# Liupeter01/Software-Rasterizer

Measured on AMD Instinct MI355X. Metric: frames_per_sec, higher is better.
Workload: dtype f32

## Files before the change

software-rasterizer_amd/csrc/srz_api.hip:

```cpp
#include <dlfcn.h>

#include <algorithm>
#include <cmath>
#include <cstdio>
#include <cstdlib>
#include <cstring>
#include <initializer_list>
#include <new>
#include <string>
#include <vector>

#include "srz_device.h"

using namespace srz;

namespace {
std::string g_create_error;

struct EventPair {
  hipEvent_t t0, t1, t2, t3;
  bool detailed;
};

struct BatchDesc {
// ... 82 lines not shown
  bool tris_aos = false;
  BBox *d_bbox = nullptr;
  uint16_t *d_tri_batch = nullptr;
  srz_light *d_lights = nullptr;
  uint32_t *d_pool = nullptr;
  uint32_t pool_sub_cap = 0, pool_n_sub = 1;
  bool pool_sized = false;
  uint32_t *d_pool_heads = nullptr, *h_pool_heads = nullptr;
  static constexpr int DEMAND_PARTS = 8;
  uint2 *d_tile_info = nullptr;
  uint32_t last_flags = 0;
  bool rendered = false;
  uint32_t *d_sparse_rows = nullptr;
  uint32_t *d_slow_list = nullptr, *d_slow_count = nullptr;
  uint4 *d_redo_list = nullptr;
  uint32_t fast_kinds = 0;
  bool any_generic = true;
  uint32_t *d_vis = nullptr, *d_work_count = nullptr, *d_chunk_rows = nullptr;
  uint4 *d_worklist = nullptr;
  uint64_t kind_slots = 0;
  uint32_t kind_mask = 0, n_kind_slots = 0;
  bool approx_shade = false;
  bool no_packed = false;
  uint32_t *d_band_desc = nullptr;
  uint2 *d_band_ent = nullptr;
  uint64_t total_groups = 0;
  ShadeDescG *d_sdesc = nullptr;
  DrawDesc *d_draws = nullptr;
  static constexpr int STAGE_RING = 4;
  uint8_t *d_dyn = nullptr;
// ... 110 lines not shown
  (void)hipFree(fs->d_dyn);
  (void)hipFree(fs->d_tris);
  (void)hipFree(fs->d_tri_pos);
  (void)hipFree(fs->d_bbox);
  (void)hipFree(fs->d_tri_batch);
  (void)hipFree(fs->d_pool);
  (void)hipFree(fs->d_pool_heads);
  if (fs->h_pool_heads) (void)hipHostFree(fs->h_pool_heads);
  if (fs->clear_tune.h_wgs) (void)hipHostFree(fs->clear_tune.h_wgs), fs->clear_tune.h_wgs = nullptr;
  if (fs->clear_tune.d_ctl) (void)hipFree(fs->clear_tune.d_ctl), fs->clear_tune.d_ctl = nullptr;
  (void)hipFree(fs->d_tile_info);
  (void)hipFree(fs->d_sparse_rows);
  (void)hipFree(fs->d_slow_list);
  (void)hipFree(fs->d_slow_count);
  (void)hipFree(fs->d_redo_list);
  (void)hipFree(fs->d_vis);
  (void)hipFree(fs->d_worklist);
  (void)hipFree(fs->d_work_count);
  (void)hipFree(fs->d_chunk_rows);
  (void)hipFree(fs->d_band_desc);
  (void)hipFree(fs->d_band_ent);
  (void)hipFree(fs->d_sdesc);
}

struct Pass {
  enum Kind { COLOUR, VISIBILITY, COUNTING, SIZE_ONLY, PEEL } kind = COLOUR;
  int f_begin = 0, f_count = -1;
  bool one_frame_scratch = false;
  const float *d_prev = nullptr;
  static Pass colour() { return {}; }
// ... 23 lines not shown
  a.bbox = fs->d_bbox;
  a.chunk_rows = fs->d_chunk_rows;
  a.band_desc = fs->d_band_desc;
  a.band_ent = fs->d_band_ent;
  a.tri_batch = fs->d_tri_batch;
  a.lights = fs->d_lights;
  a.pool = fs->d_pool;
  a.pool_heads = fs->d_pool_heads;
  a.pool_demand = fs->h_pool_heads;
  a.pool_sub_cap = fs->pool_sub_cap;
  a.pool_sub_mask = fs->pool_n_sub - 1u;
  a.tile_info = fs->d_tile_info;
  a.slow_list = fs->d_slow_list;
  a.slow_count = fs->d_slow_count;
  a.redo_list = fs->d_redo_list;
  a.redo_count = fs->d_slow_count + 1;
  a.force_ordered = a.force_generic = pass.kind == Pass::COUNTING ? 1u : 0u;
  a.any_ordered = any_frame_has(fs, flags_or, SRZ_ORDERED_RASTER) ? 1u : 0u, a.any_generic = fs->any_generic ? 1u : 0u;
  a.sdesc = fs->d_sdesc;
  a.vis = fs->d_vis;
  a.worklist = fs->d_worklist;
  a.kind_slots = fs->kind_slots;
  a.work_count = fs->d_work_count;
  a.work_cap = (uint32_t)(fs->n_frames < 8 ? fs->n_frames : (fs->n_frames + 7) / 8) * fs->n_local_bands * fs->tiles_x;
  a.tiles_x = fs->tiles_x;
  a.n_local_bands = fs->n_local_bands;
  a.n_frames = (uint32_t)fs->n_frames;
  a.out = d_out;
  a.local_rows = fs->local_rows;
  a.frame_stride = pass.one_frame_scratch ? 0 : 4ull * fs->local_rows * (uint64_t)fs->width;
// ... 836 lines not shown
    fs->pool_n_sub = n_sub;
    const uint64_t cap = std::min<uint64_t>((4ull * tri_off + 4096u) / n_sub + 64u, 0xfffffff0ull / n_sub);
    fs->pool_sub_cap = (uint32_t)cap;
    FS_TRY(dev_alloc((void **)&fs->d_pool, sizeof(uint32_t) * cap * n_sub));
    FS_TRY(dev_alloc((void **)&fs->d_pool_heads, sizeof(uint32_t) * CNT_STRIDE * 64));
    FS_TRY(hipHostMalloc((void **)&fs->h_pool_heads, sizeof(uint32_t) * CNT_STRIDE * 64 * srz_frameset::DEMAND_PARTS, hipHostMallocMapped | hipHostMallocCoherent));
    if (e == hipSuccess) std::memset(fs->h_pool_heads, 0, sizeof(uint32_t) * CNT_STRIDE * 64 * srz_frameset::DEMAND_PARTS);
    FS_TRY(dev_alloc((void **)&fs->clear_tune.d_ctl, sizeof(ClearCtl)));
    if (e == hipSuccess) FS_TRY(hipMemset(fs->clear_tune.d_ctl, 0, sizeof(ClearCtl)));
    FS_TRY(hipHostMalloc((void **)&fs->clear_tune.h_wgs, 64, hipHostMallocMapped | hipHostMallocCoherent));
    if (e == hipSuccess) *fs->clear_tune.h_wgs = 0u;
    FS_TRY(dev_alloc((void **)&fs->d_tile_info, sizeof(uint2) * fs->max_tiles));
    FS_TRY(dev_alloc((void **)&fs->d_slow_list, sizeof(uint32_t) * fs->max_tiles));
    FS_TRY(dev_alloc((void **)&fs->d_slow_count, 2 * sizeof(uint32_t)));
    FS_TRY(dev_alloc((void **)&fs->d_redo_list, sizeof(uint4) * fs->max_tiles));
  }
  FS_TRY(dev_alloc((void **)&fs->d_vis, sizeof(uint32_t) * (size_t)fs->max_tiles * ((size_t)TILE * TILE)));
  FS_TRY(ensure_worklists(fs));
  FS_TRY(dev_alloc((void **)&fs->d_work_count, sizeof(uint32_t) * CNT_STRIDE * N_WORK_LISTS));
  FS_TRY(dev_alloc((void **)&fs->d_sdesc, sizeof(ShadeDescG) * fs->h_batches.size()));
  std::vector<uint8_t> h_dyn(fs->dyn_bytes);
  stage_dyn(fs, h_dyn.data());
  FS_TRY(hipMemcpy(fs->d_dyn, h_dyn.data(), fs->dyn_bytes, hipMemcpyHostToDevice));
  if (tri_off) {
    if (copy_tris) FS_TRY(hipMemcpy(fs->d_tris, h_tris.data(), sizeof(srz_tri) * tri_off, hipMemcpyHostToDevice));
    if (!h_pos.empty()) FS_TRY(hipMemcpy(fs->d_tri_pos, h_pos.data(), sizeof(float) * h_pos.size(), hipMemcpyHostToDevice));
    FS_TRY(hipMemcpy(fs->d_tri_batch, h_tb.data(), sizeof(uint16_t) * tri_off, hipMemcpyHostToDevice));
  }
#undef FS_TRY
  if (e != hipSuccess) {
// ... 402 lines not shown
  if (!fs || !d_vis || !d_out) return fail(ctx, SRZ_E_INVALID, fn + ": null frameset / visibility buffer / output");
  const size_t bytes = srz_frameset_out_bytes(ctx, fs);
  if (out_bytes < bytes) return fail(ctx, SRZ_E_INVALID, fn + ": output buffer too small");
  if (!aligned<16>({d_vis, d_out})) return fail(ctx, SRZ_E_INVALID, fn + ": buffers must be 16-byte aligned");
  if (d_vis != d_out && ranges_overlap({d_vis, bytes}, {d_out, bytes}))
    return fail(ctx, SRZ_E_INVALID, fn + ": visibility buffer and output overlap partly");
  hipStream_t s;
  if (int rc = begin_pass(ctx, fs, stream, PASS_SHADING | PASS_VERTEX, &s)) return rc;
  ShadeVisArgs a{};
  fill_walk(a, fs, d_vis, d_out);
  a.tris = fs->d_tris, a.tri_batch = fs->d_tri_batch, a.lights = fs->d_lights, a.sdesc = fs->d_sdesc;
  a.frame_stride = 4ull * plane_words(fs);
  a.flags_or = flags & FRAME_FLAGS, a.in_place = d_vis == d_out ? 1u : 0u;
  a.any_generic = fs->any_generic ? 1u : 0u;
  a.redo_list = reinterpret_cast<uint32_t *>(fs->d_redo_list), a.redo_count = fs->d_slow_count + 1;
  HIP_TRY(ctx, hipMemsetAsync(a.redo_count, 0, sizeof(uint32_t), s));
  launch_shade_vis(a, fs->fast_kinds, fs->any_generic, fs->approx_shade, s);
  const srz_frameset::ClearTune &ct = fs->clear_tune;
  if (!ctx->env_clear_wgs && ct.d_ctl && !ct.done && fs->max_tiles >= 8192) launch_clear_rebase(ct.d_ctl, s);
  return end_pass(ctx);
}

size_t srz_frameset_gbuffer_bytes(const srz_ctx *ctx, const srz_frameset *fs, uint32_t what) {
  if (!fs || what == 0u || (what & ~GB_GROUPS) != 0u) return 0;
  return (size_t)fs->n_frames * gbuf_planes(what) * fs->local_rows * (size_t)fs->width * sizeof(float);
}

int srz_frameset_gbuffer(srz_ctx *ctx, srz_frameset *fs, const void *d_vis, void *d_out, size_t out_bytes, uint32_t what, uint32_t flags,
                         void *stream) {
  if (!ctx) return SRZ_E_INVALID;
// ... 2069 lines not shown
```

software-rasterizer_amd/csrc/srz_device.h:

```cpp
#pragma once
#include <hip/hip_runtime.h>
#include <stdint.h>

#include "../../include/srz.h"

namespace srz {

constexpr int TILE = 32;
constexpr int BAND = 32;
constexpr int KEY_STRIDE = TILE + 1;
constexpr int LDS_STRIDE = 32;
#ifndef SRZ_BAND_ROT
#define SRZ_BAND_ROT 5
#endif
__host__ __device__ inline int band_rot(int world) { return (SRZ_BAND_ROT % world) ? SRZ_BAND_ROT : (SRZ_BAND_ROT ? 1 : 0); }
__host__ __device__ inline int band_of(int lb, int rank, int world) {
  if (world == 1) return lb;
  int j = (rank - band_rot(world) * lb) % world;
  return lb * world + (j < 0 ? j + world : j);
}
__host__ __device__ inline int rank_of_band(int b, int world) { return (b + band_rot(world) * (b / world)) % world; }
constexpr uint32_t NO_TRI = 0xffffffffu;
constexpr uint32_t CNT_STRIDE = 32;
constexpr uint32_t FD_FAST_SHADE = 0x100u, FD_NL_SHIFT = 9;
// ... 76 lines not shown
  uint32_t *pool;
  uint32_t *pool_heads;
  uint32_t *pool_demand;
  uint32_t pool_sub_cap, pool_sub_mask;
  uint2 *tile_info;
  uint32_t *slow_list;
  uint32_t *slow_count;
  uint32_t other_streams;
  uint32_t clear_in_raster;
  uint32_t force_ordered;
  uint32_t any_ordered;
  uint32_t force_generic;
  uint32_t any_generic;
  uint4 *redo_list;
  uint32_t *redo_count;
  uint32_t *vis;
  uint4 *worklist;
  uint64_t kind_slots;
  uint32_t *work_count;
  uint32_t work_cap;
  uint32_t tiles_x, n_local_bands, n_frames;
  float *out;
  uint64_t frame_stride;
  uint32_t local_rows;
  int32_t shard_rank, shard_world;
  uint32_t flags_or;
  unsigned long long *stats;
  const uint32_t *clear_wgs_dev;
};

// ... 82 lines not shown
struct ShadeVisArgs {
  const FrameDesc *frames;
  const srz_tri *tris;
  const uint16_t *tri_batch;
  const srz_light *lights;
  const ShadeDescG *sdesc;
  const float *vis;
  float *out;
  uint64_t frame_stride;
  uint32_t local_rows, tiles_x, n_local_bands, n_frames;
  int32_t shard_rank, shard_world;
  uint32_t flags_or, in_place;
  uint32_t any_generic;
  uint32_t *redo_list;
  uint32_t *redo_count;
};
void launch_shade_vis(const ShadeVisArgs &a, uint32_t kinds, bool any_generic, bool approx, hipStream_t s);
struct GbufArgs {
  const FrameDesc *frames;
  const srz_tri *tris;
  const uint16_t *tri_batch;
  const ShadeDescG *sdesc;
  const float *vis;
  float *out;
  uint64_t vis_stride;
  uint64_t frame_stride;
  uint32_t local_rows, tiles_x, n_local_bands, n_frames;
  int32_t shard_rank, shard_world;
  uint32_t flags_or, what;
};
// ... 443 lines not shown
```

software-rasterizer_amd/csrc/srz_kernels.hip:

```cpp
#include "srz_device.h"

#include <algorithm>
#include <cstdio>
#include <cstdlib>
#include <type_traits>

#pragma clang fp contract(off)

namespace srz {

#define SRZ_CAS __attribute__((address_space(4)))
template <typename T> __device__ __forceinline__ const SRZ_CAS T *as_const(const T *p) { return (const SRZ_CAS T *)(p); }
typedef float f32x4 __attribute__((ext_vector_type(4)));
typedef unsigned int u32x2 __attribute__((ext_vector_type(2)));
typedef unsigned int u32x4 __attribute__((ext_vector_type(4)));

__device__ __forceinline__ float sse_max(float a, float b) { return a > b ? a : b; }
__device__ __forceinline__ float sse_min(float a, float b) { return a < b ? a : b; }
__device__ __forceinline__ float std_max(float a, float b) { return (a < b) ? b : a; }
__device__ __forceinline__ float std_clamp(float v, float lo, float hi) { return (v < lo) ? lo : (hi < v) ? hi : v; }
__device__ __forceinline__ float fmsubf(float a, float b, float c) { return __builtin_fmaf(a, b, -c); }
__device__ __forceinline__ float fmaf_(float a, float b, float c) { return __builtin_fmaf(a, b, c); }

__device__ __forceinline__ uint32_t f2u_(float f) { return __builtin_bit_cast(uint32_t, f); }
// ... 2263 lines not shown

#ifndef SRZ_FAST_MINW
#define SRZ_FAST_MINW 6
#endif
#ifndef SRZ_STAGE_TRIS
#define SRZ_STAGE_TRIS 96
#endif
constexpr uint32_t STAGE_TRIS = SRZ_STAGE_TRIS, STAGE_SD = 16;
static_assert(SRZ_STAGE_TRIS * 6 * 16 >= 2 * 32 * 32 * 4, "SRZ_STAGE_TRIS: s_tri must hold a tile's 1024 {pixel, index} pairs (>= 86 triangles)");
#ifndef SRZ_GENPOW_MINW
#define SRZ_GENPOW_MINW 5
#endif
#ifndef SRZ_SHADE_MINW
#define SRZ_SHADE_MINW 4
#endif
template <bool STATS, int FASTNL, bool BUMPY = false, bool APPROX = false>
__global__ __launch_bounds__(256, (FASTNL > 0 && FASTNL <= 2 && !BUMPY) ? SRZ_FAST_MINW : (FASTNL < 0 && FASTNL >= -2) ? SRZ_GENPOW_MINW
                                  : ((FASTNL == 3 || FASTNL == -3) && !BUMPY) ? 5 : SRZ_SHADE_MINW)
void k_shade(RenderArgs a) {
  constexpr bool FAST = FASTNL != 0, GENPOW = FASTNL < 0;
  static_assert(FAST || !BUMPY, "BUMPY is a property of the FAST builds");
  static_assert(!APPROX || (FASTNL > 0 && !BUMPY && !STATS), "the tolerance mode has FAST builds for 1..4 lights only");
  static_assert(!(GENPOW && BUMPY), "frames with BUMP / DISPLACEMENT batches and a non-integer exponent take the generic build");
  __shared__ __attribute__((aligned(16))) float s_c[3][TILE * TILE];
  __shared__ __attribute__((aligned(16))) uint32_t s_ent[PIX_SLOT];
  __shared__ uint32_t s_wcnt[4];
  __shared__ __attribute__((aligned(16))) f32x4 s_tri[STAGE_TRIS * 6];
  __shared__ uint16_t s_bat[STAGE_TRIS];
  __shared__ __attribute__((aligned(16))) ShadeDescG s_sd[STAGE_SD];
  __shared__ uint32_t s_flag;

  const int tid = threadIdx.x, lane = tid & 63;
  const int wave = __builtin_amdgcn_readfirstlane(tid >> 6);
  unsigned long long n_vis = 0, n_vis_tex = 0;
#ifdef SRZ_PHASE_PROBE
  unsigned long long ph[6] = {0, 0, 0, 0, 0, 0}, ph_t = 0;
  const unsigned long long ph_c0 = __builtin_amdgcn_s_memtime(), ph_r0 = __builtin_amdgcn_s_memrealtime();
#define SRZ_STAMP(K) { const unsigned long long t_ = __builtin_amdgcn_s_memtime(); ph[K] += t_ - ph_t, ph_t = t_; }
#else
#define SRZ_STAMP(K)
#endif

  auto shade_tile = [&](const u32x4 x, auto mode_c) {
    constexpr int MODE = decltype(mode_c)::value;
    int tid = (int)threadIdx.x;
    asm volatile("" : "+v"(tid));
    const int lane = tid & 63;
#ifdef SRZ_PHASE_PROBE
    ph_t = __builtin_amdgcn_s_memtime(), ph[5] += 1;
#endif
    const SRZ_CAS RenderArgs *ap = (const SRZ_CAS RenderArgs *)__builtin_amdgcn_kernarg_segment_ptr();
    asm volatile("" : "+s"(ap));
    const uint32_t tpf = ap->n_local_bands * ap->tiles_x;
    const bool by_lp = (x.y & WORK_LP) != 0u, staged = by_lp && x.z <= STAGE_TRIS;
    const bool lp8 = (x.y & WORK_LP8) != 0u;
    const SRZ_CAS uint32_t *tlist = as_const(ap->pool) + x.w;
    const int ly = wave * 8 + (lane >> 3), lx4 = (lane & 7) * 4;
    const int p0 = ly * TILE + lx4;
// ... 41 lines not shown
    float *out0 = ap->out + (size_t)f * ap->frame_stride + row0 * (size_t)W;

    const bool sd_mine = sd_staged && (uint32_t)tid < fd->n_batches;
    ShadeDescG sd_reg;
    sd_reg.shader = 0, sd_reg.tw = sd_reg.th = 1, sd_reg._pad = 0, sd_reg.tex = nullptr;
    if (sd_mine) {
      const SRZ_CAS ShadeDescG *g = sdesc + tid;
      sd_reg.shader = g->shader, sd_reg.tw = g->tw, sd_reg.th = g->th, sd_reg.tex = g->tex;
    }

    const int y = ty0 + ly, x4 = tx0 + lx4;
    const bool in_tile = y <= ty1 && x4 <= tx1;
    const bool full = in_tile && ((W & 3) == 0) && x4 + 3 <= tx1;
    float *gz = out0 + (size_t)ly * W + x4;
    float4 C0 = make_float4(0.f, 0.f, 0.f, 0.f), C1 = C0, C2 = C0;
    if (!fused) {
      if (full) {
        C0 = *reinterpret_cast<const float4 *>(gz + plane);
        C1 = *reinterpret_cast<const float4 *>(gz + 2 * plane);
        C2 = *reinterpret_cast<const float4 *>(gz + 3 * plane);
      } else if (in_tile) {
        if (x4 + 0 <= tx1) C0.x = gz[plane + 0], C1.x = gz[2 * plane + 0], C2.x = gz[3 * plane + 0];
        if (x4 + 1 <= tx1) C0.y = gz[plane + 1], C1.y = gz[2 * plane + 1], C2.y = gz[3 * plane + 1];
        if (x4 + 2 <= tx1) C0.z = gz[plane + 2], C1.z = gz[2 * plane + 2], C2.z = gz[3 * plane + 2];
        if (x4 + 3 <= tx1) C0.w = gz[plane + 3], C1.w = gz[2 * plane + 3], C2.w = gz[3 * plane + 3];
      }
    }
    *reinterpret_cast<float4 *>(&s_c[0][p0]) = C0;
    *reinterpret_cast<float4 *>(&s_c[1][p0]) = C1;
    *reinterpret_cast<float4 *>(&s_c[2][p0]) = C2;
#ifdef SRZ_PHASE_PROBE
    asm volatile("" : "+v"(id_raw.x), "+v"(id_raw.y), "+v"(ti[0]));
    SRZ_STAMP(0)
#endif
    uint32_t idk[4] = {id_raw.x, id_raw.y, id_raw.z, id_raw.w};
    if (lp8)
      idk[0] = id_raw.x & 0xffu, idk[1] = (id_raw.x >> 8) & 0xffu, idk[2] = (id_raw.x >> 16) & 0xffu, idk[3] = id_raw.x >> 24;
    else if (by_lp)
      idk[0] = id_raw.x & 0xffffu, idk[1] = id_raw.x >> 16, idk[2] = id_raw.y & 0xffffu, idk[3] = id_raw.y >> 16;
    uint32_t cnt2 = 0;
#pragma unroll
    for (int k = 0; k < 4; ++k) cnt2 += idk[k] == none ? 0u : ((idk[k] & sbit) ? 0x10000u : 1u);
    const uint32_t incl2 = wave_scan_add(cnt2);
    if (lane == 63) s_wcnt[wave] = incl2;
    if (tid == 0) s_flag = 0;
// ... 31 lines not shown
        const bool own = idk[k] != none, isS = own && (idk[k] & sbit) != 0;
        const uint32_t o = isS ? oS : oV, owner = idk[k] & ~sbit;
        if (own) {
          if (by_lp)
            s_ent[o] = (uint32_t)(p0 + k) | (owner << PIX_BITS);
          else
            s_ent2[2 * o] = (uint32_t)(p0 + k), s_ent2[2 * o + 1] = owner;
        }
        oV += (own && !isS) ? 1u : 0u, oS += isS ? 1u : 0u;
      }
    }
    __builtin_amdgcn_s_waitcnt(0x0f70);
    __syncthreads();
    SRZ_STAMP(2)

    const uint32_t cV = (nV + 63) >> 6, cS = (nS + 63) >> 6;
    auto class_pass = [&](auto policy, auto is_v, auto staged_c, bool count) -> bool {
      using M = decltype(policy);
      constexpr bool isV = decltype(is_v)::value, STAGED = decltype(staged_c)::value;
      bool bad = false;
      FrameK K;
      K.eye[0] = fd->eye[0], K.eye[1] = fd->eye[1], K.eye[2] = fd->eye[2];
      K.ka[0] = fd->ka[0], K.ka[1] = fd->ka[1], K.ka[2] = fd->ka[2];
      K.ks[0] = fd->ks[0], K.ks[1] = fd->ks[1], K.ks[2] = fd->ks[2];
      K.p = fd->p, K.kh = fd->kh, K.kn = fd->kn, K.n_lights = fd->n_lights;
      K.grey = (fd->flags & FD_GREY) != 0u;
      K.lights = as_const(ap->lights) + fd->light_off;
      for (uint32_t c = (uint32_t)wave; c < cV + cS; c += 4) {
        if ((c >= cS) != isV) continue;
        const uint32_t i = (isV ? c - cS : c) * 64 + lane;
        if (i >= (isV ? nV : nS)) continue;
        const uint32_t slot = isV ? i : nV + i;
        uint32_t p, id;
        if (by_lp) {
          const uint32_t en = s_ent[slot];
          p = en & PIX_MASK, id = en >> PIX_BITS;
        } else {
          p = s_ent2[2 * slot], id = s_ent2[2 * slot + 1];
        }
        float r0 = 1.f, r1 = 2.f, r2 = 3.f;
        ShadeDesc sd;
        TriFetch tf;
        const f32x4 *late = nullptr;
        if constexpr (STAGED) {
          late = s_tri + id * 6u;
          tf.batch = s_bat[id];
        } else {
// ... 41 lines not shown
            }
          }
        } else {
          if (sd_staged) {
            const ShadeDescG &g = s_sd[tf.batch];
            sd.shader = g.shader, sd.tw = g.tw, sd.th = g.th, sd.tex = as_const(g.tex);
          } else {
            const SRZ_CAS ShadeDescG *g = sdesc + tf.batch;
            sd.shader = g->shader, sd.tw = g->tw, sd.th = g->th, sd.tex = as_const(g->tex);
          }
          if constexpr (isV)
            shade_pixel_v<M>(m, K, sd, tf, late, px, py, r0, r1, r2);
          else
            shade_pixel_s<M>(m, K, sd, tf, late, px, py, r0, r1, r2);
        }
        if constexpr (std::is_same<M, FastMath>::value) bad |= m.is_bad();
        s_c[0][p] = r0, s_c[1][p] = r1, s_c[2][p] = r2;
        if (STATS && count)
          n_vis++, n_vis_tex += (sd.shader == SRZ_SHADER_TEXTURE || sd.shader == SRZ_SHADER_DISPLACEMENT || sd.shader == SRZ_SHADER_BUMP);
      }
      return bad;
    };
    auto dense_passes = [&](auto policy, bool count) -> bool {
      bool bv, bs;
      if (staged) {
        bv = class_pass(policy, std::true_type{}, std::true_type{}, count);
        bs = class_pass(policy, std::false_type{}, std::true_type{}, count);
      } else {
        bv = class_pass(policy, std::true_type{}, std::false_type{}, count);
        bs = class_pass(policy, std::false_type{}, std::false_type{}, count);
      }
      return bv | bs;
    };
    bool skip_write = false;
    if constexpr (APPROX) {
      dense_passes(ApproxMath{}, true);
      __syncthreads();
    } else if constexpr (MODE == 2) {
      if (STATS && tid == 0) atomicAdd(&ap->stats[ST_DBG_IEEE_TILES], 1ull);
      dense_passes(IeeeMath{}, true);
      __syncthreads();
    } else {
      const bool bad = dense_passes(FastMath{}, true);
      if (__ballot(bad) != 0ull && lane == 0) s_flag = 1u;
      __syncthreads();
      if (s_flag) {
        if constexpr (MODE == 0) {
          if (tid == 0) ap->redo_list[atomicAdd(ap->redo_count, 1u)] = make_uint4(x.x, x.y, x.z, x.w);
          skip_write = true;
        } else {
          if (STATS && tid == 0) atomicAdd(&ap->stats[ST_DBG_IEEE_TILES], 1ull);
          dense_passes(IeeeMath{}, false);
          __syncthreads();
        }
      }
    }

    SRZ_STAMP(3)
    if (!skip_write) {
      C0 = *reinterpret_cast<const float4 *>(&s_c[0][p0]);
      C1 = *reinterpret_cast<const float4 *>(&s_c[1][p0]);
      C2 = *reinterpret_cast<const float4 *>(&s_c[2][p0]);
// ... 20 lines not shown
  while (w < n_work) {
    const u32x4 xc = x;
    w += gridDim.x >> 3;
    if (w < n_work) x = list[w];
    if constexpr (FAST)
      shade_tile(xc, std::integral_constant<int, 0>{});
    else
      shade_tile(xc, std::integral_constant<int, 1>{});
    __syncthreads();
  }

  if constexpr (!FAST) {
    const uint32_t n_redo = *as_const(a.redo_count);
    for (uint32_t i = blockIdx.x; i < n_redo; i += gridDim.x) {
      const u32x4 xr = reinterpret_cast<const SRZ_CAS u32x4 *>(as_const(a.redo_list))[i];
      shade_tile(xr, std::integral_constant<int, 2>{});
      __syncthreads();
    }

  }
#ifdef SRZ_PHASE_PROBE
  if (lane == 0 && FAST) {
    for (int k = 0; k < 6; ++k)
      if (ph[k]) atomicAdd(&a.stats[ST_DBG_CYC_A + k], ph[k]);
    atomicAdd(&a.stats[0], __builtin_amdgcn_s_memtime() - ph_c0), atomicAdd(&a.stats[1], __builtin_amdgcn_s_memrealtime() - ph_r0);
  }
#endif
  if (STATS) {
    for (int o = 32; o > 0; o >>= 1) {
      n_vis += __shfl_down(n_vis, o);
      n_vis_tex += __shfl_down(n_vis_tex, o);
    }
    if (lane == 0) {
      if (n_vis) atomicAdd(&a.stats[ST_VISIBLE], n_vis);
// ... 182 lines not shown
}

template <int FASTNL, bool BUMPY = false, bool APPROX = false>
__global__ __launch_bounds__(256, FASTNL == -4 ? 3 : SRZ_SHADE_MINW) void k_shade_vis(ShadeVisArgs a) {
  constexpr bool FAST = FASTNL != 0;
  static_assert(FAST || !BUMPY, "BUMPY is a property of the FAST builds");
  static_assert(!APPROX || (FASTNL > 0 && !BUMPY), "the tolerance mode has FAST builds for 1..4 lights only");
  constexpr uint32_t KIND = build_kind<FASTNL, BUMPY>();
  __shared__ __attribute__((aligned(16))) float s_in[3][TILE * TILE];
  __shared__ __attribute__((aligned(16))) float s_c[3][TILE * TILE];
  __shared__ uint32_t s_idx[PIX_SLOT];
  __shared__ uint16_t s_pix[PIX_SLOT];
  __shared__ uint32_t s_wcnt[4];
  __shared__ uint32_t s_flag;
  __shared__ uint8_t s_bog[256];
  const int tid = threadIdx.x, lane = tid & 63;
  const int wave = __builtin_amdgcn_readfirstlane(tid >> 6);
  const int p0 = tid * 4;
  const uint32_t tpf = a.n_local_bands * a.tiles_x;
  auto shade_tile = [&](const uint32_t f, const uint32_t t, auto mode_c) {
    constexpr int MODE = decltype(mode_c)::value;
    const PassTile pt = pass_tile(a, f, t);
    const SRZ_CAS FrameDesc *fd = pt.fd;
    const int tx0 = pt.rc.tx0, ty0 = pt.rc.ty0, tx1 = pt.rc.tx1, x4 = pt.x4;
    const bool in_tile = pt.inside, whole = pt.whole, fused = pt.fused(a.flags_or);
    const size_t plane = pt.rc.plane;
    const float *gv = a.vis + (size_t)f * a.frame_stride + pt.poff;
    float *go = pt.out;
    uint32_t id[4], bogus = 0u;
    const uint32_t own = quad_ids(pt, gv, id, &bogus);
    s_bog[tid] = (uint8_t)bogus;
    const bool any_own = own != 0u;
    float4 in[3] = {make_float4(0.f, 0.f, 0.f, 0.f), make_float4(0.f, 0.f, 0.f, 0.f), make_float4(0.f, 0.f, 0.f, 0.f)};
    if (any_own) {
      if (whole) {
// ... 2 lines not shown
        in[2] = *reinterpret_cast<const float4 *>(gv + 3 * plane);
      } else {
#pragma unroll
        for (int k = 0; k < 4; ++k)
          if (x4 + k <= tx1) quad_at(in[0], k) = gv[k], quad_at(in[1], k) = gv[2 * plane + k], quad_at(in[2], k) = gv[3 * plane + k];
      }
    }
#pragma unroll
    for (int i = 0; i < 3; ++i) *reinterpret_cast<float4 *>(&s_in[i][p0]) = in[i];
    uint32_t cnt2 = 0;
#pragma unroll
    for (int k = 0; k < 4; ++k) cnt2 += id[k] == 0u ? 0u : ((id[k] & S_CLASS_BIT) ? 0x10000u : 1u);
    const uint32_t incl2 = wave_scan_add(cnt2);
    if (lane == 63) s_wcnt[wave] = incl2;
    if (tid == 0) s_flag = 0u;
    __syncthreads();
    uint32_t bV = 0, bS = 0, nV = 0, nS = 0;
#pragma unroll
    for (int w2 = 0; w2 < 4; ++w2) {
      const uint32_t t2 = s_wcnt[w2];
      bV += w2 < wave ? (t2 & 0xffffu) : 0u, bS += w2 < wave ? (t2 >> 16) : 0u, nV += t2 & 0xffffu, nS += t2 >> 16;
    }
    nV = (uint32_t)__builtin_amdgcn_readfirstlane((int)nV), nS = (uint32_t)__builtin_amdgcn_readfirstlane((int)nS);
    {
      uint32_t oV = bV + ((incl2 - cnt2) & 0xffffu), oS = nV + bS + ((incl2 - cnt2) >> 16);
#pragma unroll
      for (int k = 0; k < 4; ++k) {
        if (id[k] == 0u) continue;
        const bool isS = (id[k] & S_CLASS_BIT) != 0u;
        const uint32_t o = isS ? oS++ : oV++;
        s_idx[o] = (id[k] & ~S_CLASS_BIT) - 1u, s_pix[o] = (uint16_t)(p0 + k);
      }
    }
    __syncthreads();
    if (nV + nS != 0u) {
      const SRZ_CAS srz_tri *tris = as_const(a.tris) + fd->tri_off;
      const SRZ_CAS uint16_t *tri_batch = as_const(a.tri_batch) + fd->tri_off;
      const SRZ_CAS ShadeDescG *sdesc = as_const(a.sdesc) + fd->batch_off;
      const uint32_t cV = (nV + 63) >> 6, cS = (nS + 63) >> 6;
      auto class_pass = [&](auto policy, auto is_v, auto gen_c) -> bool {
        using M = decltype(policy);
        constexpr bool isV = decltype(is_v)::value, GEN = decltype(gen_c)::value;
        bool bad = false;
        const FrameK K = frame_k(fd, as_const(a.lights));
        for (uint32_t c = (uint32_t)wave; c < cV + cS; c += 4) {
          if ((c >= cS) != isV) continue;
          const uint32_t i = (isV ? c - cS : c) * 64 + lane;
          if (i >= (isV ? nV : nS)) continue;
          const uint32_t slot = isV ? i : nV + i;
          const uint32_t idx = s_idx[slot], p = s_pix[slot];
          TriFetch tf;
          const SRZ_CAS f32x4 *tq = reinterpret_cast<const SRZ_CAS f32x4 *>(tris + idx);
          const F3 n0 = ld3(reinterpret_cast<const SRZ_CAS float *>(tq) + 9);
          tf.q2 = f32x4{0.f, n0.x, n0.y, n0.z}, tf.q3 = tq[3], tf.q4 = tq[4], tf.q5 = tq[5];
          tf.batch = tri_batch[idx];
          TriAttr at;
          unpack_attr(tf, at);
          const float zz = s_in[0][p], alpha = s_in[1][p], beta = s_in[2][p];
          const float gamma = isV ? 1.0f - (alpha + beta) : 1.0f - alpha - beta;
          const float fx = (float)(tx0 + (int)(p & 31u)), fy = (float)(ty0 + (int)(p >> 5));
          float r0 = 1.f, r1 = 2.f, r2 = 3.f;
          M m;
          ShadeDesc sd;
          if constexpr (!GEN) {
// ... 21 lines not shown
                    run(std::integral_constant<int, SRZ_SHADER_BUMP>{});
                  else
                    run(std::integral_constant<int, SRZ_SHADER_DISPLACEMENT>{});
                }
                todo = false;
              }
            }
          } else {
            const SRZ_CAS ShadeDescG *g = sdesc + tf.batch;
            sd.shader = g->shader, sd.tw = g->tw, sd.th = g->th, sd.tex = as_const(g->tex);
            if constexpr (isV)
              shade_bary_v<M, -1, 0>(m, K, sd, at, alpha, beta, gamma, fx, fy, zz, r0, r1, r2);
            else
              shade_bary_s<M, -1, 0>(m, K, sd, at, alpha, beta, gamma, fx, fy, zz, r0, r1, r2);
          }
          if constexpr (std::is_same<M, FastMath>::value) bad |= m.is_bad();
          s_c[0][p] = r0, s_c[1][p] = r1, s_c[2][p] = r2;
        }
        return bad;
      };
      auto dense_passes = [&](auto policy, auto gen_c) -> bool {
        const bool bv = class_pass(policy, std::true_type{}, gen_c);
        const bool bs = class_pass(policy, std::false_type{}, gen_c);
        return bv | bs;
      };
      if constexpr (APPROX) {
        dense_passes(ApproxMath{}, std::false_type{});
      } else if constexpr (MODE == 2) {
        dense_passes(IeeeMath{}, std::true_type{});
      } else {
        const bool bad = dense_passes(FastMath{}, std::integral_constant<bool, MODE == 1>{});
        if (__ballot(bad) != 0ull && lane == 0) s_flag = 1u;
        __syncthreads();
        if (s_flag) {
          if constexpr (MODE == 0) {
            if (tid == 0) a.redo_list[atomicAdd(a.redo_count, 1u)] = f * tpf + t;
            __syncthreads();
            return;
          } else {
            dense_passes(IeeeMath{}, std::true_type{});
          }
        }
      }
      __syncthreads();
    }
    const uint32_t bog = (a.in_place && fused) ? (uint32_t)s_bog[tid] : 0u;
    if (in_tile && (any_own || (fused && !a.in_place) || bog != 0u)) {
      const bool own4 = own == 15u;
      float4 q[4];
      q[0] = *reinterpret_cast<const float4 *>(&s_in[0][p0]);
#pragma unroll
      for (int i = 0; i < 3; ++i) q[i + 1] = *reinterpret_cast<const float4 *>(&s_c[i][p0]);
#pragma unroll
      for (int k = 0; k < 4; ++k)
        if (!(own & (1u << k))) {
          quad_at(q[0], k) = __builtin_inff();
#pragma unroll
          for (int i = 1; i < 4; ++i) quad_at(q[i], k) = 0.f;
        }
      if (a.in_place) {
        if (own4) {
          const float4 c[3] = {q[1], q[2], q[3]};
// ... 8 lines not shown
#pragma unroll
              for (int i = 0; i < 4; ++i) go[i * plane + k] = quad_at(q[i], k);
            }
          }
        }
      } else if (fused || own4) {
        quad_store(go, plane, q, whole, x4, tx1);
      } else {
#pragma unroll
        for (int k = 0; k < 4; ++k)
          if (own & (1u << k))
#pragma unroll
            for (int i = 0; i < 4; ++i) go[i * plane + k] = quad_at(q[i], k);
      }
    }
    __syncthreads();
  };

  if (FAST || a.any_generic)
    pass_tiles(a, [&](uint32_t f, uint32_t t) {
      if (frame_kind(as_const(a.frames)[f].flags) != KIND) return;
      shade_tile(f, t, std::integral_constant<int, FAST ? 0 : 1>{});
    });
  if constexpr (!FAST) {
    const uint32_t n_redo = *as_const(a.redo_count);
    for (uint32_t i = blockIdx.x; i < n_redo; i += gridDim.x) {
      const uint32_t it = as_const(a.redo_list)[i];
      shade_tile(it / tpf, it % tpf, std::integral_constant<int, 2>{});
    }
  }
}

typedef float f32x2 __attribute__((ext_vector_type(2)));
struct GbufPixel {
  float n[3], uv[2], kd[3];
  uint32_t batch1;
};
__device__ __forceinline__ GbufPixel gbuf_pixel(uint32_t what, uint32_t id, float alpha, float beta, const SRZ_CAS srz_tri *tris,
                                                const SRZ_CAS uint16_t *tri_batch, const SRZ_CAS ShadeDescG *sdesc) {
  GbufPixel o = {{0.f, 0.f, 0.f}, {0.f, 0.f}, {1.f, 1.f, 1.f}, 0u};
  IeeeMath m;
  const bool isS = (id & S_CLASS_BIT) != 0u;
  const uint32_t idx = (id & ~S_CLASS_BIT) - 1u;
// ... 4577 lines not shown
  launch_kind<3, true>(kinds, approx, launch), launch_kind<4, true>(kinds, approx, launch);
  launch_kind<-1, false>(kinds, approx, launch), launch_kind<-2, false>(kinds, approx, launch);
  launch_kind<-3, false>(kinds, approx, launch), launch_kind<-4, false>(kinds, approx, launch);
}

void launch_shade(const RenderArgs &a, uint32_t max_tiles, bool stats, uint32_t kinds, bool any_generic, bool approx, hipStream_t s) {
  if (max_tiles == 0) return;
  const dim3 grid = shade_grid(a, max_tiles);
  if (stats) {
    hipLaunchKernelGGL((k_shade<true, 0>), grid, dim3(256), 0, s, a);
    return;
  }
  launch_fast_kinds(kinds, approx, [&](auto nl, auto bumpy, auto ap) {
    hipLaunchKernelGGL((k_shade<false, decltype(nl)::value, decltype(bumpy)::value, decltype(ap)::value>), grid, dim3(256), 0, s, a);
  });
  dim3 ggrid(any_generic ? grid.x : (grid.x < 128u ? grid.x : 128u));
  hipLaunchKernelGGL((k_shade<false, 0>), ggrid, dim3(256), 0, s, a);
}

void launch_visibility(const RenderArgs &a, uint32_t max_tiles, hipStream_t s) {
  if (max_tiles == 0) return;
  hipLaunchKernelGGL(k_visibility, shade_grid(a, max_tiles), dim3(256), 0, s, a);
}

void launch_shade_vis(const ShadeVisArgs &a, uint32_t kinds, bool any_generic, bool approx, hipStream_t s) {
  const uint32_t items = a.n_frames * a.n_local_bands * a.tiles_x;
  if (items == 0) return;
  const dim3 grid(tile_grid(items)), blk(256);
  launch_fast_kinds(kinds, approx, [&](auto nl, auto bumpy, auto ap) {
    hipLaunchKernelGGL((k_shade_vis<decltype(nl)::value, decltype(bumpy)::value, decltype(ap)::value>), grid, blk, 0, s, a);
  });
// ... 347 lines not shown
```

Baseline: 329,600.

## Redo only flagged pixels via per-tile bitmask instead of re-shading whole tiles

```diff
diff --git a/software-rasterizer_amd/csrc/srz_api.hip b/software-rasterizer_amd/csrc/srz_api.hip
--- a/software-rasterizer_amd/csrc/srz_api.hip
+++ b/software-rasterizer_amd/csrc/srz_api.hip
@@ -120,6 +120,7 @@
   uint32_t *d_sparse_rows = nullptr;
   uint32_t *d_slow_list = nullptr, *d_slow_count = nullptr;
   uint4 *d_redo_list = nullptr;
+  uint32_t *d_redo_mask = nullptr;
   uint32_t fast_kinds = 0;
   bool any_generic = true;
   uint32_t *d_vis = nullptr, *d_work_count = nullptr, *d_chunk_rows = nullptr;
@@ -260,6 +261,7 @@
   (void)hipFree(fs->d_slow_list);
   (void)hipFree(fs->d_slow_count);
   (void)hipFree(fs->d_redo_list);
+  (void)hipFree(fs->d_redo_mask);
   (void)hipFree(fs->d_vis);
   (void)hipFree(fs->d_worklist);
   (void)hipFree(fs->d_work_count);
@@ -313,6 +315,7 @@
   a.slow_list = fs->d_slow_list;
   a.slow_count = fs->d_slow_count;
   a.redo_list = fs->d_redo_list;
+  a.redo_mask = fs->d_redo_mask;
   a.redo_count = fs->d_slow_count + 1;
   a.force_ordered = a.force_generic = pass.kind == Pass::COUNTING ? 1u : 0u;
   a.any_ordered = any_frame_has(fs, flags_or, SRZ_ORDERED_RASTER) ? 1u : 0u, a.any_generic = fs->any_generic ? 1u : 0u;
@@ -1179,6 +1182,7 @@
     FS_TRY(dev_alloc((void **)&fs->d_slow_list, sizeof(uint32_t) * fs->max_tiles));
     FS_TRY(dev_alloc((void **)&fs->d_slow_count, 2 * sizeof(uint32_t)));
     FS_TRY(dev_alloc((void **)&fs->d_redo_list, sizeof(uint4) * fs->max_tiles));
+    FS_TRY(dev_alloc((void **)&fs->d_redo_mask, sizeof(uint32_t) * REDO_MASK_WORDS * fs->max_tiles));
   }
   FS_TRY(dev_alloc((void **)&fs->d_vis, sizeof(uint32_t) * (size_t)fs->max_tiles * ((size_t)TILE * TILE)));
   FS_TRY(ensure_worklists(fs));
@@ -1611,6 +1615,7 @@
   a.flags_or = flags & FRAME_FLAGS, a.in_place = d_vis == d_out ? 1u : 0u;
   a.any_generic = fs->any_generic ? 1u : 0u;
   a.redo_list = reinterpret_cast<uint32_t *>(fs->d_redo_list), a.redo_count = fs->d_slow_count + 1;
+  a.redo_mask = fs->d_redo_mask;
   HIP_TRY(ctx, hipMemsetAsync(a.redo_count, 0, sizeof(uint32_t), s));
   launch_shade_vis(a, fs->fast_kinds, fs->any_generic, fs->approx_shade, s);
   const srz_frameset::ClearTune &ct = fs->clear_tune;
diff --git a/software-rasterizer_amd/csrc/srz_device.h b/software-rasterizer_amd/csrc/srz_device.h
--- a/software-rasterizer_amd/csrc/srz_device.h
+++ b/software-rasterizer_amd/csrc/srz_device.h
@@ -8,6 +8,7 @@
 
 constexpr int TILE = 32;
 constexpr int BAND = 32;
+constexpr uint32_t REDO_MASK_WORDS = TILE * TILE / 32;
 constexpr int KEY_STRIDE = TILE + 1;
 constexpr int LDS_STRIDE = 32;
 #ifndef SRZ_BAND_ROT
@@ -114,6 +115,7 @@
   uint32_t any_generic;
   uint4 *redo_list;
   uint32_t *redo_count;
+  uint32_t *redo_mask;
   uint32_t *vis;
   uint4 *worklist;
   uint64_t kind_slots;
@@ -226,6 +228,7 @@
   uint32_t any_generic;
   uint32_t *redo_list;
   uint32_t *redo_count;
+  uint32_t *redo_mask;
 };
 void launch_shade_vis(const ShadeVisArgs &a, uint32_t kinds, bool any_generic, bool approx, hipStream_t s);
 struct GbufArgs {
diff --git a/software-rasterizer_amd/csrc/srz_kernels.hip b/software-rasterizer_amd/csrc/srz_kernels.hip
--- a/software-rasterizer_amd/csrc/srz_kernels.hip
+++ b/software-rasterizer_amd/csrc/srz_kernels.hip
@@ -2301,6 +2301,26 @@
 #ifndef SRZ_SHADE_MINW
 #define SRZ_SHADE_MINW 4
 #endif
+__device__ __forceinline__ void redo_mark(uint32_t *s_mask, uint32_t p) {
+  asm volatile("" : "+v"(p));
+  atomicOr(&s_mask[p >> 5], 1u << (p & 31u));
+}
+__device__ __forceinline__ bool redo_marked(const uint32_t *s_mask, uint32_t p) { return ((s_mask[p >> 5] >> (p & 31u)) & 1u) != 0u; }
+template <class E>
+__device__ __forceinline__ void redo_hand_back(E *list, uint32_t *count, uint32_t *gmask, uint32_t *s_mask, const E &entry, int lane) {
+  uint32_t slot = 0u;
+  if (lane == 0) slot = atomicAdd(count, 1u), list[slot] = entry;
+  slot = (uint32_t)__builtin_amdgcn_readfirstlane((int)slot);
+  if (lane < (int)REDO_MASK_WORDS) gmask[(size_t)slot * REDO_MASK_WORDS + lane] = s_mask[lane], s_mask[lane] = 0u;
+}
+__device__ __forceinline__ void redo_patch_begin(uint32_t *s_mask, uint32_t *s_npatch, const uint32_t *gmask, uint32_t slot, int tid) {
+  if (tid < (int)REDO_MASK_WORDS) s_mask[tid] = as_const(gmask)[(size_t)slot * REDO_MASK_WORDS + tid];
+  if (tid < 2) s_npatch[tid] = 0u;
+}
+__device__ __forceinline__ void redo_patch_collect(const uint32_t *s_mask, uint32_t *s_npatch, uint32_t *s_list, uint32_t slot, uint32_t p, bool is_v) {
+  if (redo_marked(s_mask, p)) s_list[(is_v ? 0u : PIX_SLOT) + atomicAdd(&s_npatch[is_v ? 0 : 1], 1u)] = slot;
+}
+
 template <bool STATS, int FASTNL, bool BUMPY = false, bool APPROX = false>
 __global__ __launch_bounds__(256, (FASTNL > 0 && FASTNL <= 2 && !BUMPY) ? SRZ_FAST_MINW : (FASTNL < 0 && FASTNL >= -2) ? SRZ_GENPOW_MINW
                                   : ((FASTNL == 3 || FASTNL == -3) && !BUMPY) ? 5 : SRZ_SHADE_MINW)
@@ -2316,9 +2336,13 @@
   __shared__ uint16_t s_bat[STAGE_TRIS];
   __shared__ __attribute__((aligned(16))) ShadeDescG s_sd[STAGE_SD];
   __shared__ uint32_t s_flag;
+  __shared__ uint32_t s_mask[REDO_MASK_WORDS];
+  __shared__ uint32_t s_npatch[2];
+  constexpr bool PATCHES = !STATS;
 
   const int tid = threadIdx.x, lane = tid & 63;
   const int wave = __builtin_amdgcn_readfirstlane(tid >> 6);
+  if (FASTNL != 0 && PATCHES && tid < (int)REDO_MASK_WORDS) s_mask[tid] = 0u;
   unsigned long long n_vis = 0, n_vis_tex = 0;
 #ifdef SRZ_PHASE_PROBE
   unsigned long long ph[6] = {0, 0, 0, 0, 0, 0}, ph_t = 0;
@@ -2328,7 +2352,7 @@
 #define SRZ_STAMP(K)
 #endif
 
-  auto shade_tile = [&](const u32x4 x, auto mode_c) {
+  auto shade_tile = [&](const u32x4 x, auto mode_c, const uint32_t ri = 0u) {
     constexpr int MODE = decltype(mode_c)::value;
     int tid = (int)threadIdx.x;
     asm volatile("" : "+v"(tid));
@@ -2400,7 +2424,8 @@
     const bool full = in_tile && ((W & 3) == 0) && x4 + 3 <= tx1;
     float *gz = out0 + (size_t)ly * W + x4;
     float4 C0 = make_float4(0.f, 0.f, 0.f, 0.f), C1 = C0, C2 = C0;
-    if (!fused) {
+    if constexpr (MODE == 3) redo_patch_begin(s_mask, s_npatch, ap->redo_mask, ri, tid);
+    if (MODE != 3 && !fused) {
       if (full) {
         C0 = *reinterpret_cast<const float4 *>(gz + plane);
         C1 = *reinterpret_cast<const float4 *>(gz + 2 * plane);
@@ -2412,9 +2437,11 @@
         if (x4 + 3 <= tx1) C0.w = gz[plane + 3], C1.w = gz[2 * plane + 3], C2.w = gz[3 * plane + 3];
       }
     }
-    *reinterpret_cast<float4 *>(&s_c[0][p0]) = C0;
-    *reinterpret_cast<float4 *>(&s_c[1][p0]) = C1;
-    *reinterpret_cast<float4 *>(&s_c[2][p0]) = C2;
+    if constexpr (MODE != 3) {
+      *reinterpret_cast<float4 *>(&s_c[0][p0]) = C0;
+      *reinterpret_cast<float4 *>(&s_c[1][p0]) = C1;
+      *reinterpret_cast<float4 *>(&s_c[2][p0]) = C2;
+    }
 #ifdef SRZ_PHASE_PROBE
     asm volatile("" : "+v"(id_raw.x), "+v"(id_raw.y), "+v"(ti[0]));
     SRZ_STAMP(0)
@@ -2476,7 +2503,15 @@
     __syncthreads();
     SRZ_STAMP(2)
 
-    const uint32_t cV = (nV + 63) >> 6, cS = (nS + 63) >> 6;
+    uint32_t *const s_patch = reinterpret_cast<uint32_t *>(&s_c[0][0]);
+    uint32_t nVc = nV, nSc = nS;
+    if constexpr (MODE == 3) {
+      for (uint32_t sl = (uint32_t)tid; sl < nV + nS; sl += 256u)
+        redo_patch_collect(s_mask, s_npatch, s_patch, sl, by_lp ? (s_ent[sl] & PIX_MASK) : s_ent2[2 * sl], sl < nV);
+      __syncthreads();
+      nVc = (uint32_t)__builtin_amdgcn_readfirstlane((int)s_npatch[0]), nSc = (uint32_t)__builtin_amdgcn_readfirstlane((int)s_npatch[1]);
+    }
+    const uint32_t cV = (nVc + 63) >> 6, cS = (nSc + 63) >> 6;
     auto class_pass = [&](auto policy, auto is_v, auto staged_c, bool count) -> bool {
       using M = decltype(policy);
       constexpr bool isV = decltype(is_v)::value, STAGED = decltype(staged_c)::value;
@@ -2491,8 +2526,9 @@
       for (uint32_t c = (uint32_t)wave; c < cV + cS; c += 4) {
         if ((c >= cS) != isV) continue;
         const uint32_t i = (isV ? c - cS : c) * 64 + lane;
-        if (i >= (isV ? nV : nS)) continue;
-        const uint32_t slot = isV ? i : nV + i;
+        if (i >= (isV ? nVc : nSc)) continue;
+        uint32_t slot = isV ? i : nV + i;
+        if constexpr (MODE == 3) slot = s_patch[isV ? i : PIX_SLOT + i];
         uint32_t p, id;
         if (by_lp) {
           const uint32_t en = s_ent[slot];
@@ -2564,8 +2600,18 @@
           else
             shade_pixel_s<M>(m, K, sd, tf, late, px, py, r0, r1, r2);
         }
-        if constexpr (std::is_same<M, FastMath>::value) bad |= m.is_bad();
-        s_c[0][p] = r0, s_c[1][p] = r1, s_c[2][p] = r2;
+        if constexpr (std::is_same<M, FastMath>::value) {
+          const bool b = m.is_bad();
+          bad |= b;
+          if constexpr (MODE == 0 && PATCHES)
+            if (b) redo_mark(s_mask, p);
+        }
+        if constexpr (MODE == 3) {
+          float *g = out0 + (size_t)(p >> 5) * W + px;
+          if (px <= tx1 && py <= ty1) g[plane] = r0, g[2 * plane] = r1, g[3 * plane] = r2;
+        } else {
+          s_c[0][p] = r0, s_c[1][p] = r1, s_c[2][p] = r2;
+        }
         if (STATS && count)
           n_vis++, n_vis_tex += (sd.shader == SRZ_SHADER_TEXTURE || sd.shader == SRZ_SHADER_DISPLACEMENT || sd.shader == SRZ_SHADER_BUMP);
       }
@@ -2582,7 +2628,7 @@
       }
       return bv | bs;
     };
-    bool skip_write = false;
+    bool skip_write = MODE == 3;
     if constexpr (APPROX) {
       dense_passes(ApproxMath{}, true);
       __syncthreads();
@@ -2590,12 +2636,16 @@
       if (STATS && tid == 0) atomicAdd(&ap->stats[ST_DBG_IEEE_TILES], 1ull);
       dense_passes(IeeeMath{}, true);
       __syncthreads();
+    } else if constexpr (MODE == 3) {
+      dense_passes(IeeeMath{}, false);
     } else {
       const bool bad = dense_passes(FastMath{}, true);
       if (__ballot(bad) != 0ull && lane == 0) s_flag = 1u;
       __syncthreads();
       if (s_flag) {
-        if constexpr (MODE == 0) {
+        if constexpr (MODE == 0 && PATCHES) {
+          if (wave == 0) redo_hand_back(ap->redo_list, ap->redo_count, ap->redo_mask, s_mask, make_uint4(x.x, x.y, x.z, x.w), lane);
+        } else if constexpr (MODE == 0) {
           if (tid == 0) ap->redo_list[atomicAdd(ap->redo_count, 1u)] = make_uint4(x.x, x.y, x.z, x.w);
           skip_write = true;
         } else {
@@ -2646,10 +2696,9 @@
     const uint32_t n_redo = *as_const(a.redo_count);
     for (uint32_t i = blockIdx.x; i < n_redo; i += gridDim.x) {
       const u32x4 xr = reinterpret_cast<const SRZ_CAS u32x4 *>(as_const(a.redo_list))[i];
-      shade_tile(xr, std::integral_constant<int, 2>{});
+      shade_tile(xr, std::integral_constant<int, PATCHES ? 3 : 2>{}, i);
       __syncthreads();
     }
-
   }
 #ifdef SRZ_PHASE_PROBE
   if (lane == 0 && FAST) {
@@ -2862,11 +2911,14 @@
   __shared__ uint32_t s_wcnt[4];
   __shared__ uint32_t s_flag;
   __shared__ uint8_t s_bog[256];
+  __shared__ uint32_t s_mask[REDO_MASK_WORDS];
+  __shared__ uint32_t s_npatch[2];
   const int tid = threadIdx.x, lane = tid & 63;
   const int wave = __builtin_amdgcn_readfirstlane(tid >> 6);
   const int p0 = tid * 4;
   const uint32_t tpf = a.n_local_bands * a.tiles_x;
-  auto shade_tile = [&](const uint32_t f, const uint32_t t, auto mode_c) {
+  if (FAST && tid < (int)REDO_MASK_WORDS) s_mask[tid] = 0u;
+  auto shade_tile = [&](const uint32_t f, const uint32_t t, auto mode_c, const uint32_t ri = 0u) {
     constexpr int MODE = decltype(mode_c)::value;
     const PassTile pt = pass_tile(a, f, t);
     const SRZ_CAS FrameDesc *fd = pt.fd;
@@ -2899,6 +2951,7 @@
     const uint32_t incl2 = wave_scan_add(cnt2);
     if (lane == 63) s_wcnt[wave] = incl2;
     if (tid == 0) s_flag = 0u;
+    if constexpr (MODE == 3) redo_patch_begin(s_mask, s_npatch, a.redo_mask, ri, tid);
     __syncthreads();
     uint32_t bV = 0, bS = 0, nV = 0, nS = 0;
 #pragma unroll
@@ -2922,7 +2975,14 @@
       const SRZ_CAS srz_tri *tris = as_const(a.tris) + fd->tri_off;
       const SRZ_CAS uint16_t *tri_batch = as_const(a.tri_batch) + fd->tri_off;
       const SRZ_CAS ShadeDescG *sdesc = as_const(a.sdesc) + fd->batch_off;
-      const uint32_t cV = (nV + 63) >> 6, cS = (nS + 63) >> 6;
+      uint32_t *const s_patch = reinterpret_cast<uint32_t *>(&s_c[0][0]);
+      uint32_t nVc = nV, nSc = nS;
+      if constexpr (MODE == 3) {
+        for (uint32_t sl = (uint32_t)tid; sl < nV + nS; sl += 256u) redo_patch_collect(s_mask, s_npatch, s_patch, sl, s_pix[sl], sl < nV);
+        __syncthreads();
+        nVc = (uint32_t)__builtin_amdgcn_readfirstlane((int)s_npatch[0]), nSc = (uint32_t)__builtin_amdgcn_readfirstlane((int)s_npatch[1]);
+      }
+      const uint32_t cV = (nVc + 63) >> 6, cS = (nSc + 63) >> 6;
       auto class_pass = [&](auto policy, auto is_v, auto gen_c) -> bool {
         using M = decltype(policy);
         constexpr bool isV = decltype(is_v)::value, GEN = decltype(gen_c)::value;
@@ -2931,8 +2991,9 @@
         for (uint32_t c = (uint32_t)wave; c < cV + cS; c += 4) {
           if ((c >= cS) != isV) continue;
           const uint32_t i = (isV ? c - cS : c) * 64 + lane;
-          if (i >= (isV ? nV : nS)) continue;
-          const uint32_t slot = isV ? i : nV + i;
+          if (i >= (isV ? nVc : nSc)) continue;
+          uint32_t slot = isV ? i : nV + i;
+          if constexpr (MODE == 3) slot = s_patch[isV ? i : PIX_SLOT + i];
           const uint32_t idx = s_idx[slot], p = s_pix[slot];
           TriFetch tf;
           const SRZ_CAS f32x4 *tq = reinterpret_cast<const SRZ_CAS f32x4 *>(tris + idx);
@@ -2984,8 +3045,20 @@
             else
               shade_bary_s<M, -1, 0>(m, K, sd, at, alpha, beta, gamma, fx, fy, zz, r0, r1, r2);
           }
-          if constexpr (std::is_same<M, FastMath>::value) bad |= m.is_bad();
-          s_c[0][p] = r0, s_c[1][p] = r1, s_c[2][p] = r2;
+          uint32_t pm = p;
+          asm volatile("" : "+v"(pm), "+v"(r0));
+          if constexpr (std::is_same<M, FastMath>::value) {
+            const bool b = m.is_bad();
+            bad |= b;
+            if constexpr (MODE == 0)
+              if (b) redo_mark(s_mask, pm);
+          }
+          if constexpr (MODE == 3) {
+            float *g = pt.rc.out0 + (size_t)(pm >> 5) * (size_t)fd->width + (size_t)(tx0 + (int)(pm & 31u));
+            g[plane] = r0, g[2 * plane] = r1, g[3 * plane] = r2;
+          } else {
+            s_c[0][pm] = r0, s_c[1][pm] = r1, s_c[2][pm] = r2;
+          }
         }
         return bad;
       };
@@ -2996,26 +3069,20 @@
       };
       if constexpr (APPROX) {
         dense_passes(ApproxMath{}, std::false_type{});
-      } else if constexpr (MODE == 2) {
+      } else if constexpr (MODE == 2 || MODE == 3) {
         dense_passes(IeeeMath{}, std::true_type{});
       } else {
         const bool bad = dense_passes(FastMath{}, std::integral_constant<bool, MODE == 1>{});
         if (__ballot(bad) != 0ull && lane == 0) s_flag = 1u;
         __syncthreads();
-        if (s_flag) {
-          if constexpr (MODE == 0) {
-            if (tid == 0) a.redo_list[atomicAdd(a.redo_count, 1u)] = f * tpf + t;
-            __syncthreads();
-            return;
-          } else {
-            dense_passes(IeeeMath{}, std::true_type{});
-          }
-        }
+        if constexpr (MODE == 1)
+          if (s_flag) dense_passes(IeeeMath{}, std::true_type{});
       }
       __syncthreads();
     }
     const uint32_t bog = (a.in_place && fused) ? (uint32_t)s_bog[tid] : 0u;
-    if (in_tile && (any_own || (fused && !a.in_place) || bog != 0u)) {
+    const bool flagged = MODE == 0 && s_flag != 0u;
+    if (MODE != 3 && !(flagged && a.in_place) && in_tile && (any_own || (fused && !a.in_place) || bog != 0u)) {
       const bool own4 = own == 15u;
       float4 q[4];
       q[0] = *reinterpret_cast<const float4 *>(&s_in[0][p0]);
@@ -3054,6 +3121,12 @@
             for (int i = 0; i < 4; ++i) go[i * plane + k] = quad_at(q[i], k);
       }
     }
+    if constexpr (MODE == 0)
+      if (flagged && wave == 0) {
+        int l = lane;
+        asm volatile("" : "+v"(l));
+        redo_hand_back(a.redo_list, a.redo_count, a.redo_mask, s_mask, f * tpf + t, l);
+      }
     __syncthreads();
   };
 
@@ -3066,7 +3139,10 @@
     const uint32_t n_redo = *as_const(a.redo_count);
     for (uint32_t i = blockIdx.x; i < n_redo; i += gridDim.x) {
       const uint32_t it = as_const(a.redo_list)[i];
-      shade_tile(it / tpf, it % tpf, std::integral_constant<int, 2>{});
+      if (a.in_place)
+        shade_tile(it / tpf, it % tpf, std::integral_constant<int, 2>{});
+      else
+        shade_tile(it / tpf, it % tpf, std::integral_constant<int, 3>{}, i);
     }
   }
 }
@@ -7674,7 +7750,7 @@
   launch_fast_kinds(kinds, approx, [&](auto nl, auto bumpy, auto ap) {
     hipLaunchKernelGGL((k_shade<false, decltype(nl)::value, decltype(bumpy)::value, decltype(ap)::value>), grid, dim3(256), 0, s, a);
   });
-  dim3 ggrid(any_generic ? grid.x : (grid.x < 128u ? grid.x : 128u));
+  dim3 ggrid(any_generic ? grid.x : (grid.x < 1024u ? grid.x : 1024u));
   hipLaunchKernelGGL((k_shade<false, 0>), ggrid, dim3(256), 0, s, a);
 }
 
```

Result: no change. 329,800 (median of 3 runs) (+0.1%).
